# dash-robotics/perception

Measured on AMD Instinct MI355X. Metric: frames/sec (640x480 D435 cloud, plane+cluster+ICP), higher is better.
Workload: dtype f32

## Files before the change

### perception_amd/csrc/k_icp_lat.hip

```cpp
#include "kernels.hpp"
#include "icp_solve_row.hpp"
#include "lat_search.hpp"

namespace cd {

#ifdef CD_LAT_TIMERS
__device__ unsigned long long g_lat_stats[8];
extern "C" int cd_debug_lat_stats(unsigned long long* out, int reset) {
    if (hipMemcpyFromSymbol(out, HIP_SYMBOL(g_lat_stats), sizeof(g_lat_stats)) != hipSuccess) return -1;
    if (reset) { unsigned long long z[8] = {0}; (void)hipMemcpyToSymbol(HIP_SYMBOL(g_lat_stats), z, sizeof(z)); }
    return 0;
}
#define LAT_T(k) { const long long tn_ = clock64(); tph[k] += tn_ - tlast; tlast = tn_; }
#else
#define LAT_T(k)
#endif

struct LatSlot {
    int k, src_off, n, tslot;
    int phase;
    int gen;
    int ready;
    int pad;
};
enum { LAT_ITER = 0, LAT_FIT = 1, LAT_EMPTY = 2 };

#ifndef CD_LAT_SOLVE_ROW
#define CD_LAT_SOLVE_ROW 1
#endif
#ifndef CD_LAT_WAVES_PER_EU
#define CD_LAT_WAVES_PER_EU 4
#endif
template <int CPW, int WPC, bool BOUNDED>
__global__ void __launch_bounds__(CPW * WPC * WAVE, CD_LAT_WAVES_PER_EU)
k_icp_lat(int nitems, const int* __restrict__ order, const IcpCluster* __restrict__ cl, IcpState* __restrict__ st,
          unsigned long long* __restrict__ accf, const IcpLattice* __restrict__ lats, float4* __restrict__ src,
          const float4* __restrict__ src0, int* __restrict__ queue, unsigned long long* __restrict__ busy,
          unsigned long long* __restrict__ busy_out, IcpParams prm, IcpBound bnd) {
    __shared__ float4 s_tab[CPW][LAT_MAX_TAB];
    __shared__ int4 s_face[CPW][2 * LAT_MAX_FACES];
    __shared__ unsigned long long s_acc[CPW][16];
    __shared__ IcpState s_so[CPW];
    __shared__ LatSlot s_slot[CPW];
    __shared__ int s_flags[2];
    __shared__ unsigned s_nv[BOUNDED ? CPW : 1];
    const int lane = threadIdx.x & 63, wave = threadIdx.x >> 6;
    const int slot = wave / WPC, sub = wave % WPC;
    const long long wg_t0 = wall_clock64();
    auto refill = [&](int s) {
        LatSlot& sl = s_slot[s];
        for (int i = 0; i < 16; ++i) s_acc[s][i] = 0ull;
        if constexpr (BOUNDED) s_nv[s] = 0u;
        sl.ready = 0;
        for (;;) {
            const int item = atomicAdd(queue, 1);
            if (item >= nitems) { sl.phase = LAT_EMPTY; return; }
            const int k = order[item];
            if (st[2 * (size_t)k].done) continue;
            const IcpCluster c = cl[k];
            sl.k = k; sl.src_off = c.src_off; sl.n = c.n; sl.tslot = c.slot;
            s_so[s] = st[2 * (size_t)k];
            sl.phase = LAT_ITER;
            sl.gen += 1;
            return;
        }
    };
    if (threadIdx.x < CPW) { s_slot[threadIdx.x].gen = 0; refill(threadIdx.x); }
    if (threadIdx.x == 0) { s_flags[0] = 0; s_flags[1] = 1; }
    __syncthreads();
    int my_gen = 0;
#ifdef CD_LAT_TIMERS
    long long tph[6] = {0, 0, 0, 0, 0, 0}, tlast = clock64();
#endif
    for (;;) {
        if (s_flags[1]) {
            const LatSlot sl = s_slot[slot];
            const bool mine = sl.phase != LAT_EMPTY && sl.gen != my_gen;
            if (mine) {
                const IcpLattice* __restrict__ L = lats + sl.tslot;
                for (int i = sub * WAVE + lane; i < L->ntab; i += WPC * WAVE) s_tab[slot][i] = L->tab[i];
                if (sub == 0 && lane < LAT_MAX_FACES) {
                    const int f = lane, w = L->w[f], u = L->fast[f], v = 3 - w - u;
                    s_face[slot][f] = make_int4(w, u, L->base[f], __float_as_int(L->c[f]));
                    s_face[slot][LAT_MAX_FACES + f] = make_int4(L->toff[u], L->toff[v < 0 || v > 2 ? 0 : v], L->n[u], 0);
                }
                my_gen = sl.gen;
            }
            __syncthreads();
        }
        LAT_T(5)
        {
            const int phase = __builtin_amdgcn_readfirstlane(s_slot[slot].phase), n = __builtin_amdgcn_readfirstlane(s_slot[slot].n);
            const int src_off = __builtin_amdgcn_readfirstlane(s_slot[slot].src_off), tslot = __builtin_amdgcn_readfirstlane(s_slot[slot].tslot);
            const int npass = (n + 63) >> 6;
            float4* pts = src + src_off;
            const float4* tab = s_tab[slot];
            const int4* face = s_face[slot];
            LatFaces F;
            {
                const IcpLattice* __restrict__ L = lats + (phase == LAT_EMPTY ? 0 : tslot);
                lat_faces_load(L, F);
            }
            const bool nf3 = F.nface <= 3;
            if (phase == LAT_ITER) {
                const bool moved = s_so[slot].iters > 0;
                float T[12];
#pragma unroll
                for (int i = 0; i < 12; ++i) T[i] = s_so[slot].T[i];
                unsigned long long S[16];
#pragma unroll
                for (int i = 0; i < 16; ++i) S[i] = 0ull;
                unsigned nv = 0u;
                float4 pnext = pts[min((sub << 6) + lane, n - 1)];
                for (int pss = sub; pss < npass; pss += WPC) {
                    const int myq = (pss << 6) + lane;
                    const bool act = myq < n;
                    const float4 p = pnext;
                    pnext = pts[min(((pss + WPC) << 6) + lane, n - 1)];
                    float px = p.x, py = p.y, pz = p.z;
                    if (moved) {
                        xform(T, p.x, p.y, p.z, px, py, pz);
                        if (act) pts[myq] = make_float4(px, py, pz, p.w);
                    }
                    const LatHit h = F.axes ? lat_nearest_axes<true>(tab, face, F, px, py, pz)
                                            : (nf3 ? lat_nearest<true, 3>(tab, face, F, px, py, pz) : lat_nearest<true, LAT_MAX_FACES>(tab, face, F, px, py, pz));
                    const bool keep = act && (!BOUNDED || h.d <= bnd.d2_max);
                    if constexpr (BOUNDED) nv += (unsigned)__popcll(ballot64(keep));
                    if (keep) {
                        const float pv[3] = {px, py, pz}, qv[3] = {h.nx, h.ny, h.nz};
                        const float big_c = fmaxf(fmaxf(fmaxf(fabsf(px), fabsf(py)), fabsf(pz)), fmaxf(fmaxf(fabsf(h.nx), fabsf(h.ny)), fabsf(h.nz)));
                        if (big_c < 256.f && h.d < 16384.f) {
#pragma unroll
                            for (int a = 0; a < 3; ++a) {
                                S[a] += LatFix<FIX_SHIFT>::bits(pv[a]);
                                S[3 + a] += LatFix<FIX_SHIFT>::bits(qv[a]);
#pragma unroll
                                for (int b = 0; b < 3; ++b) S[6 + 3 * a + b] += LatFix<FIX_SHIFT>::bits(__fmul_rn(qv[a], pv[b]));
                            }
                            S[15] += LatFix<FIX_SHIFT_D2>::bits(h.d);
                        } else {
#pragma unroll
                            for (int a = 0; a < 3; ++a) {
                                S[a] += (unsigned long long)fixq(pv[a], FIX_SHIFT) + LatFix<FIX_SHIFT>::C;
                                S[3 + a] += (unsigned long long)fixq(qv[a], FIX_SHIFT) + LatFix<FIX_SHIFT>::C;
#pragma unroll
                                for (int b = 0; b < 3; ++b) S[6 + 3 * a + b] += (unsigned long long)fixq(__fmul_rn(qv[a], pv[b]), FIX_SHIFT) + LatFix<FIX_SHIFT>::C;
                            }
                            S[15] += (unsigned long long)fixq(h.d, FIX_SHIFT_D2) + LatFix<FIX_SHIFT_D2>::C;
                        }
                    }
                }
                if (sub < npass) wave_fold_to_lds(S, 16, s_acc[slot]);
                if constexpr (BOUNDED) { if (sub < npass && lane == 0) atomicAdd(&s_nv[slot], nv); }
                if (sub == 0 && lane == 0) s_slot[slot].ready = 1;
            } else if (phase == LAT_FIT) {
                const float4* pts0 = src0 + src_off;
                float T[12], Tf[12];
#pragma unroll
                for (int i = 0; i < 12; ++i) {
                    T[i] = __int_as_float(__builtin_amdgcn_readfirstlane(__float_as_int(s_so[slot].T[i])));
                    Tf[i] = __int_as_float(__builtin_amdgcn_readfirstlane(__float_as_int(s_so[slot].Tfinal[i])));
                }
                unsigned long long S[16];
#pragma unroll
                for (int i = 0; i < 16; ++i) S[i] = 0ull;
                float4 pnext = pts[min((sub << 6) + lane, n - 1)], p0next = pts0[min((sub << 6) + lane, n - 1)];
                for (int pss = sub; pss < npass; pss += WPC) {
                    const int myq = (pss << 6) + lane;
                    const bool act = myq < n;
                    const float4 p = pnext, p0 = p0next;
                    pnext = pts[min(((pss + WPC) << 6) + lane, n - 1)];
                    p0next = pts0[min(((pss + WPC) << 6) + lane, n - 1)];
                    float ox, oy, oz;
                    xform(T, p.x, p.y, p.z, ox, oy, oz);
                    if (act) pts[myq] = make_float4(ox, oy, oz, p.w);
                    float qx, qy, qz;
                    xform(Tf, p0.x, p0.y, p0.z, qx, qy, qz);
                    const LatHit h = F.axes ? lat_nearest_axes<false>(tab, face, F, qx, qy, qz)
                                            : (nf3 ? lat_nearest<false, 3>(tab, face, F, qx, qy, qz) : lat_nearest<false, LAT_MAX_FACES>(tab, face, F, qx, qy, qz));
                    if (act) S[0] += h.d < 16384.f ? LatFix<FIX_SHIFT_D2>::bits(h.d) : (unsigned long long)fixq(h.d, FIX_SHIFT_D2) + LatFix<FIX_SHIFT_D2>::C;
                }
                if (sub < npass) wave_fold_to_lds(S, 1, s_acc[slot]);
            }
        }
        LAT_T(0)
        if (threadIdx.x == 0) s_flags[1] = 0;
        __syncthreads();
        LAT_T(1)
#if CD_LAT_SOLVE_ROW
        const int tid = (int)threadIdx.x | s_flags[0];
        if (tid < CPW * 16) {
            const int s = tid >> 4, l = tid & 15;
            LatSlot& sl = s_slot[s];
            const int phase = sl.phase, ready = sl.ready;
            const int nv = BOUNDED && phase == LAT_ITER ? (int)s_nv[s] : sl.n;
            const unsigned long long off = (unsigned long long)nv * LatFix<FIX_SHIFT>::C, off_d = (unsigned long long)nv * LatFix<FIX_SHIFT_D2>::C;
            if (phase == LAT_ITER && ready) {
                RowLanes row(tid);
                RowLanes::V<unsigned long long> a;
                a.v = s_acc[s][l] - (l == 15 ? off_d : off);
                const int done = icp_step_row<BOUNDED>(row, s_so[s], a, nv, prm);
                s_acc[s][l] = 0ull;
                if (l == 0) {
                    if (done) sl.phase = LAT_FIT;
                    if constexpr (BOUNDED) s_nv[s] = 0u;
                    sl.ready = 0;
                }
            } else if (phase == LAT_FIT && l == 0) {
                s_so[s].done = 1;
                st[2 * (size_t)sl.k] = s_so[s];
                st[2 * (size_t)sl.k + 1] = s_so[s];
                accf[sl.k] = s_acc[s][0] - off_d;
                refill(s);
                if (sl.phase != LAT_EMPTY) s_flags[1] = 1;
            }
        }
#else
        if (threadIdx.x < CPW) {
            const int s = threadIdx.x;
            LatSlot& sl = s_slot[s];
            const int nv = BOUNDED && sl.phase == LAT_ITER ? (int)s_nv[s] : sl.n;
            const unsigned long long off = (unsigned long long)nv * LatFix<FIX_SHIFT>::C, off_d = (unsigned long long)nv * LatFix<FIX_SHIFT_D2>::C;
            if (sl.phase == LAT_ITER && sl.ready) {
                for (int i = 0; i < 15; ++i) s_acc[s][i] -= off;
                s_acc[s][15] -= off_d;
                if (icp_step<BOUNDED>(s_so[s], s_acc[s], nv, prm)) sl.phase = LAT_FIT;
                for (int i = 0; i < 16; ++i) s_acc[s][i] = 0ull;
                if constexpr (BOUNDED) s_nv[s] = 0u;
                sl.ready = 0;
            } else if (sl.phase == LAT_FIT) {
                s_so[s].done = 1;
                st[2 * (size_t)sl.k] = s_so[s];
                st[2 * (size_t)sl.k + 1] = s_so[s];
                accf[sl.k] = s_acc[s][0] - off_d;
                refill(s);
                if (sl.phase != LAT_EMPTY) s_flags[1] = 1;
            }
        }
#endif
        LAT_T(2)
        __syncthreads();
        LAT_T(3)
#ifdef CD_LAT_TIMERS
        tph[4] += 1;
#endif
        int all_empty = 1;
#pragma unroll
        for (int s = 0; s < CPW; ++s) all_empty &= s_slot[s].phase == LAT_EMPTY ? 1 : 0;
        if (all_empty) break;
    }
#ifdef CD_LAT_TIMERS
    if (threadIdx.x == 0) for (int i = 0; i < 6; ++i) atomicAdd(&g_lat_stats[i], (unsigned long long)tph[i]);
#endif
    if (threadIdx.x == 0 && busy) {
        atomicAdd(busy, (unsigned long long)(wall_clock64() - wg_t0) * (unsigned long long)(CPW * WPC));
        if (busy_out) {
            __threadfence();
            if (atomicAdd(queue + 1, 1) == (int)gridDim.x - 1) {
                __threadfence();
                *busy_out = atomicAdd(busy, 0ull);
            }
        }
    }
}

__device__ __forceinline__ bool lat_same_bits(float a, float b) { return __float_as_uint(a) == __float_as_uint(b); }

__global__ void __launch_bounds__(BLOCK) k_lat_nn(const IcpLattice* __restrict__ L, const float4* __restrict__ q, int n, int* __restrict__ out_idx,
                                                  float* __restrict__ out_d2) {
    __shared__ float4 s_tab[LAT_MAX_TAB];
    __shared__ int4 s_face[2 * LAT_MAX_FACES];
    LatFaces F;
    lat_stage<BLOCK>(L, F, s_tab, s_face);
    for (int base = blockIdx.x * BLOCK; base < n; base += gridDim.x * BLOCK) {
        const int i = base + threadIdx.x;
        const float4 p = q[i < n ? i : n - 1];
        const LatHit h = lat_nearest<true, LAT_MAX_FACES, true>(s_tab, s_face, F, p.x, p.y, p.z);
        const LatHit g = lat_nearest<false, 3>(s_tab, s_face, F, p.x, p.y, p.z);
        bool same = F.nface > 3 || h.d == g.d;
        const int idx = lat_index(s_face, F, h);
        if (F.axes) {
            const LatHit a = lat_nearest_axes<true, true>(s_tab, s_face, F, p.x, p.y, p.z);
            const LatHit b = lat_nearest_axes<false>(s_tab, s_face, F, p.x, p.y, p.z);
            same = same && a.d == h.d && b.d == h.d && lat_same_bits(a.nx, h.nx) && lat_same_bits(a.ny, h.ny) && lat_same_bits(a.nz, h.nz) &&
                   lat_index(s_face, F, a) == idx;
        }
        if (i < n) { out_idx[i] = idx; out_d2[i] = same ? h.d : __uint_as_float(0x7fc00000u); }
    }
}

template <int CPW, int WPC>
static void launch_lat_shape(hipStream_t s, int nitems, int n_wg, const int* order, const IcpCluster* cl, IcpState* st, unsigned long long* accf,
                             const IcpLattice* lats, float4* src, const float4* src0, int* queue, unsigned long long* busy, unsigned long long* busy_out,
                             IcpParams prm, const IcpBound& bnd) {
    if (bnd.bounded)
        hipLaunchKernelGGL((k_icp_lat<CPW, WPC, true>), dim3(n_wg), dim3(CPW * WPC * WAVE), 0, s, nitems, order, cl, st, accf, lats, src, src0, queue, busy, busy_out, prm, bnd);
    else
        hipLaunchKernelGGL((k_icp_lat<CPW, WPC, false>), dim3(n_wg), dim3(CPW * WPC * WAVE), 0, s, nitems, order, cl, st, accf, lats, src, src0, queue, busy, busy_out, prm, bnd);
}
void launch_icp_lat(hipStream_t s, int nitems, int cpw, int wpc, int n_wg, const IcpProblems& P, const IcpTemplates& T, const IcpScratch& S,
                    unsigned long long* busy, unsigned long long* busy_out, IcpParams prm, const IcpBound& bnd) {
    if (nitems <= 0 || n_wg <= 0) return;
#define CD_LAT_CASE(C, W) if (cpw == C && wpc == W) return launch_lat_shape<C, W>(s, nitems, n_wg, P.order, P.cl, P.st, P.accf, T.lats, S.src, S.src0, S.queue, busy, busy_out, prm, bnd);
    CD_LAT_CASE(1, 1) CD_LAT_CASE(1, 2) CD_LAT_CASE(1, 4) CD_LAT_CASE(1, 8) CD_LAT_CASE(1, 16)
    CD_LAT_CASE(2, 1) CD_LAT_CASE(2, 2) CD_LAT_CASE(2, 4)
    CD_LAT_CASE(4, 1) CD_LAT_CASE(4, 2) CD_LAT_CASE(4, 4)
    CD_LAT_CASE(8, 1) CD_LAT_CASE(8, 2)
#undef CD_LAT_CASE
    launch_lat_shape<1, 4>(s, nitems, n_wg, P.order, P.cl, P.st, P.accf, T.lats, S.src, S.src0, S.queue, busy, busy_out, prm, bnd);
}
void launch_lat_nn(hipStream_t s, const IcpLattice* lat, const float4* q, int n, int* out_idx, float* out_d2) {
    if (n <= 0) return;
    const int g = (n + BLOCK - 1) / BLOCK;
    hipLaunchKernelGGL(k_lat_nn, dim3(g < 1024 ? g : 1024), dim3(BLOCK), 0, s, lat, q, n, out_idx, out_d2);
}

}
```

Baseline: 209,900.

## Balance lattice ICP passes across all waves in the workgroup instead of per slot

Replaces the fixed mapping, where each slot owned WPC waves and those waves split only that cluster's 64-point passes, with a global partition. The total pass count across all CPW slots is split evenly across every wave in the workgroup, so a wave can cover parts of several clusters. The goal is to stop waves idling when cluster sizes differ or a slot is empty. In exchange it adds a per-iteration loop over slots, per-segment face loads and LDS folds, and drops the ready flag so the solve runs every iteration for each ITER slot.

Result: no change. 210,400, median of 5 (+0.2%).

```diff
diff --git a/perception_amd/csrc/k_icp_lat.hip b/perception_amd/csrc/k_icp_lat.hip
--- a/perception_amd/csrc/k_icp_lat.hip
+++ b/perception_amd/csrc/k_icp_lat.hip
@@ -1,6 +1,7 @@
 #include "kernels.hpp"
 #include "icp_solve_row.hpp"
 #include "lat_search.hpp"
+#include "lat_balance.hpp"
 
 namespace cd {
 
@@ -12,18 +13,20 @@
     return 0;
 }
 #define LAT_T(k) { const long long tn_ = clock64(); tph[k] += tn_ - tlast; tlast = tn_; }
+#define LAT_WAIT(stmt) { const long long tb_ = clock64(); stmt; twait += clock64() - tb_; }
 #else
 #define LAT_T(k)
+#define LAT_WAIT(stmt) stmt;
 #endif
 
 struct LatSlot {
     int k, src_off, n, tslot;
     int phase;
     int gen;
-    int ready;
-    int pad;
+    int pad[2];
 };
 enum { LAT_ITER = 0, LAT_FIT = 1, LAT_EMPTY = 2 };
+static_assert(lat_passes(LAT_ITER, 65) == 2 && lat_passes(LAT_FIT, 64) == 1 && lat_passes(LAT_EMPTY, 64) == 0, "lat_balance.hpp's phase words");
 
 #ifndef CD_LAT_SOLVE_ROW
 #define CD_LAT_SOLVE_ROW 1
@@ -46,12 +49,12 @@
     __shared__ unsigned s_nv[BOUNDED ? CPW : 1];
     const int lane = threadIdx.x & 63, wave = threadIdx.x >> 6;
     const int slot = wave / WPC, sub = wave % WPC;
+    const int wave_u = __builtin_amdgcn_readfirstlane(wave);
     const long long wg_t0 = wall_clock64();
     auto refill = [&](int s) {
         LatSlot& sl = s_slot[s];
         for (int i = 0; i < 16; ++i) s_acc[s][i] = 0ull;
         if constexpr (BOUNDED) s_nv[s] = 0u;
-        sl.ready = 0;
         for (;;) {
             const int item = atomicAdd(queue, 1);
             if (item >= nitems) { sl.phase = LAT_EMPTY; return; }
@@ -70,7 +73,7 @@
     __syncthreads();
     int my_gen = 0;
 #ifdef CD_LAT_TIMERS
-    long long tph[6] = {0, 0, 0, 0, 0, 0}, tlast = clock64();
+    long long tph[6] = {0, 0, 0, 0, 0, 0}, tlast = clock64(), twait = 0;
 #endif
     for (;;) {
         if (s_flags[1]) {
@@ -90,112 +93,123 @@
         }
         LAT_T(5)
         {
-            const int phase = __builtin_amdgcn_readfirstlane(s_slot[slot].phase), n = __builtin_amdgcn_readfirstlane(s_slot[slot].n);
-            const int src_off = __builtin_amdgcn_readfirstlane(s_slot[slot].src_off), tslot = __builtin_amdgcn_readfirstlane(s_slot[slot].tslot);
-            const int npass = (n + 63) >> 6;
-            float4* pts = src + src_off;
-            const float4* tab = s_tab[slot];
-            const int4* face = s_face[slot];
-            LatFaces F;
-            {
-                const IcpLattice* __restrict__ L = lats + (phase == LAT_EMPTY ? 0 : tslot);
-                lat_faces_load(L, F);
-            }
-            const bool nf3 = F.nface <= 3;
-            if (phase == LAT_ITER) {
-                const bool moved = s_so[slot].iters > 0;
-                float T[12];
-#pragma unroll
-                for (int i = 0; i < 12; ++i) T[i] = s_so[slot].T[i];
-                unsigned long long S[16];
-#pragma unroll
-                for (int i = 0; i < 16; ++i) S[i] = 0ull;
-                unsigned nv = 0u;
-                float4 pnext = pts[min((sub << 6) + lane, n - 1)];
-                for (int pss = sub; pss < npass; pss += WPC) {
-                    const int myq = (pss << 6) + lane;
-                    const bool act = myq < n;
-                    const float4 p = pnext;
-                    pnext = pts[min(((pss + WPC) << 6) + lane, n - 1)];
-                    float px = p.x, py = p.y, pz = p.z;
-                    if (moved) {
-                        xform(T, p.x, p.y, p.z, px, py, pz);
-                        if (act) pts[myq] = make_float4(px, py, pz, p.w);
-                    }
-                    const LatHit h = F.axes ? lat_nearest_axes<true>(tab, face, F, px, py, pz)
-                                            : (nf3 ? lat_nearest<true, 3>(tab, face, F, px, py, pz) : lat_nearest<true, LAT_MAX_FACES>(tab, face, F, px, py, pz));
-                    const bool keep = act && (!BOUNDED || h.d <= bnd.d2_max);
-                    if constexpr (BOUNDED) nv += (unsigned)__popcll(ballot64(keep));
-                    if (keep) {
-                        const float pv[3] = {px, py, pz}, qv[3] = {h.nx, h.ny, h.nz};
-                        const float big_c = fmaxf(fmaxf(fmaxf(fabsf(px), fabsf(py)), fabsf(pz)), fmaxf(fmaxf(fabsf(h.nx), fabsf(h.ny)), fabsf(h.nz)));
-                        if (big_c < 256.f && h.d < 16384.f) {
-#pragma unroll
-                            for (int a = 0; a < 3; ++a) {
-                                S[a] += LatFix<FIX_SHIFT>::bits(pv[a]);
-                                S[3 + a] += LatFix<FIX_SHIFT>::bits(qv[a]);
-#pragma unroll
-                                for (int b = 0; b < 3; ++b) S[6 + 3 * a + b] += LatFix<FIX_SHIFT>::bits(__fmul_rn(qv[a], pv[b]));
+            int P = 0;
+#pragma unroll
+            for (int s = 0; s < CPW; ++s) P += lat_passes(__builtin_amdgcn_readfirstlane(s_slot[s].phase), __builtin_amdgcn_readfirstlane(s_slot[s].n));
+            LatBalance bal(P, CPW * WPC, wave_u);
+#pragma unroll 1
+            for (int s = 0; s < CPW && (CPW == 1 || bal.base < bal.hi); ++s) {
+                const int phase = __builtin_amdgcn_readfirstlane(s_slot[s].phase), n = __builtin_amdgcn_readfirstlane(s_slot[s].n);
+                constexpr int STEP = CPW == 1 ? WPC : 1;
+                int first, end;
+                if constexpr (CPW == 1) {
+                    first = wave_u; end = lat_passes(phase, n);
+                    if (first >= end) continue;
+                } else {
+                    if (!bal.next(lat_passes(phase, n), first, end)) continue;
+                }
+                const int src_off = __builtin_amdgcn_readfirstlane(s_slot[s].src_off), tslot = __builtin_amdgcn_readfirstlane(s_slot[s].tslot);
+                float4* pts = src + src_off;
+                const float4* tab = s_tab[s];
+                const int4* face = s_face[s];
+                LatFaces F;
+                lat_faces_load(lats + tslot, F);
+                const bool nf3 = F.nface <= 3;
+                if (phase == LAT_ITER) {
+                    const bool moved = s_so[s].iters > 0;
+                    float T[12];
+#pragma unroll
+                    for (int i = 0; i < 12; ++i) T[i] = s_so[s].T[i];
+                    unsigned long long S[16];
+#pragma unroll
+                    for (int i = 0; i < 16; ++i) S[i] = 0ull;
+                    unsigned nv = 0u;
+                    float4 pnext = pts[min((first << 6) + lane, n - 1)];
+                    for (int pss = first; pss < end; pss += STEP) {
+                        const int myq = (pss << 6) + lane;
+                        const bool act = myq < n;
+                        const float4 p = pnext;
+                        pnext = pts[min(((CPW == 1 ? pss + STEP : min(pss + 1, end - 1)) << 6) + lane, n - 1)];
+                        float px = p.x, py = p.y, pz = p.z;
+                        if (moved) {
+                            xform(T, p.x, p.y, p.z, px, py, pz);
+                            if (act) pts[myq] = make_float4(px, py, pz, p.w);
+                        }
+                        const LatHit h = F.axes ? lat_nearest_axes<true>(tab, face, F, px, py, pz)
+                                                : (nf3 ? lat_nearest<true, 3>(tab, face, F, px, py, pz) : lat_nearest<true, LAT_MAX_FACES>(tab, face, F, px, py, pz));
+                        const bool keep = act && (!BOUNDED || h.d <= bnd.d2_max);
+                        if constexpr (BOUNDED) nv += (unsigned)__popcll(ballot64(keep));
+                        if (keep) {
+                            const float pv[3] = {px, py, pz}, qv[3] = {h.nx, h.ny, h.nz};
+                            const float big_c = fmaxf(fmaxf(fmaxf(fabsf(px), fabsf(py)), fabsf(pz)), fmaxf(fmaxf(fabsf(h.nx), fabsf(h.ny)), fabsf(h.nz)));
+                            if (big_c < 256.f && h.d < 16384.f) {
+#pragma unroll
+                                for (int a = 0; a < 3; ++a) {
+                                    S[a] += LatFix<FIX_SHIFT>::bits(pv[a]);
+                                    S[3 + a] += LatFix<FIX_SHIFT>::bits(qv[a]);
+#pragma unroll
+                                    for (int b = 0; b < 3; ++b) S[6 + 3 * a + b] += LatFix<FIX_SHIFT>::bits(__fmul_rn(qv[a], pv[b]));
+                                }
+                                S[15] += LatFix<FIX_SHIFT_D2>::bits(h.d);
+                            } else {
+#pragma unroll
+                                for (int a = 0; a < 3; ++a) {
+                                    S[a] += (unsigned long long)fixq(pv[a], FIX_SHIFT) + LatFix<FIX_SHIFT>::C;
+                                    S[3 + a] += (unsigned long long)fixq(qv[a], FIX_SHIFT) + LatFix<FIX_SHIFT>::C;
+#pragma unroll
+                                    for (int b = 0; b < 3; ++b) S[6 + 3 * a + b] += (unsigned long long)fixq(__fmul_rn(qv[a], pv[b]), FIX_SHIFT) + LatFix<FIX_SHIFT>::C;
+                                }
+                                S[15] += (unsigned long long)fixq(h.d, FIX_SHIFT_D2) + LatFix<FIX_SHIFT_D2>::C;
                             }
-                            S[15] += LatFix<FIX_SHIFT_D2>::bits(h.d);
-                        } else {
-#pragma unroll
-                            for (int a = 0; a < 3; ++a) {
-                                S[a] += (unsigned long long)fixq(pv[a], FIX_SHIFT) + LatFix<FIX_SHIFT>::C;
-                                S[3 + a] += (unsigned long long)fixq(qv[a], FIX_SHIFT) + LatFix<FIX_SHIFT>::C;
-#pragma unroll
-                                for (int b = 0; b < 3; ++b) S[6 + 3 * a + b] += (unsigned long long)fixq(__fmul_rn(qv[a], pv[b]), FIX_SHIFT) + LatFix<FIX_SHIFT>::C;
-                            }
-                            S[15] += (unsigned long long)fixq(h.d, FIX_SHIFT_D2) + LatFix<FIX_SHIFT_D2>::C;
                         }
                     }
+                    wave_fold_to_lds(S, 16, s_acc[s]);
+                    if constexpr (BOUNDED) { if (lane == 0) atomicAdd(&s_nv[s], nv); }
+                } else {
+                    const float4* pts0 = src0 + src_off;
+                    float T[12], Tf[12];
+#pragma unroll
+                    for (int i = 0; i < 12; ++i) {
+                        T[i] = __int_as_float(__builtin_amdgcn_readfirstlane(__float_as_int(s_so[s].T[i])));
+                        Tf[i] = __int_as_float(__builtin_amdgcn_readfirstlane(__float_as_int(s_so[s].Tfinal[i])));
+                    }
+                    unsigned long long S[16];
+#pragma unroll
+                    for (int i = 0; i < 16; ++i) S[i] = 0ull;
+                    float4 pnext = pts[min((first << 6) + lane, n - 1)], p0next = pts0[min((first << 6) + lane, n - 1)];
+                    for (int pss = first; pss < end; pss += STEP) {
+                        const int myq = (pss << 6) + lane;
+                        const bool act = myq < n;
+                        const float4 p = pnext, p0 = p0next;
+                        const int nq = min(((CPW == 1 ? pss + STEP : min(pss + 1, end - 1)) << 6) + lane, n - 1);
+                        pnext = pts[nq];
+                        p0next = pts0[nq];
+                        float ox, oy, oz;
+                        xform(T, p.x, p.y, p.z, ox, oy, oz);
+                        if (act) pts[myq] = make_float4(ox, oy, oz, p.w);
+                        float qx, qy, qz;
+                        xform(Tf, p0.x, p0.y, p0.z, qx, qy, qz);
+                        const LatHit h = F.axes ? lat_nearest_axes<false>(tab, face, F, qx, qy, qz)
+                                                : (nf3 ? lat_nearest<false, 3>(tab, face, F, qx, qy, qz) : lat_nearest<false, LAT_MAX_FACES>(tab, face, F, qx, qy, qz));
+                        if (act) S[0] += h.d < 16384.f ? LatFix<FIX_SHIFT_D2>::bits(h.d) : (unsigned long long)fixq(h.d, FIX_SHIFT_D2) + LatFix<FIX_SHIFT_D2>::C;
+                    }
+                    wave_fold_to_lds(S, 1, s_acc[s]);
                 }
-                if (sub < npass) wave_fold_to_lds(S, 16, s_acc[slot]);
-                if constexpr (BOUNDED) { if (sub < npass && lane == 0) atomicAdd(&s_nv[slot], nv); }
-                if (sub == 0 && lane == 0) s_slot[slot].ready = 1;
-            } else if (phase == LAT_FIT) {
-                const float4* pts0 = src0 + src_off;
-                float T[12], Tf[12];
-#pragma unroll
-                for (int i = 0; i < 12; ++i) {
-                    T[i] = __int_as_float(__builtin_amdgcn_readfirstlane(__float_as_int(s_so[slot].T[i])));
-                    Tf[i] = __int_as_float(__builtin_amdgcn_readfirstlane(__float_as_int(s_so[slot].Tfinal[i])));
-                }
-                unsigned long long S[16];
-#pragma unroll
-                for (int i = 0; i < 16; ++i) S[i] = 0ull;
-                float4 pnext = pts[min((sub << 6) + lane, n - 1)], p0next = pts0[min((sub << 6) + lane, n - 1)];
-                for (int pss = sub; pss < npass; pss += WPC) {
-                    const int myq = (pss << 6) + lane;
-                    const bool act = myq < n;
-                    const float4 p = pnext, p0 = p0next;
-                    pnext = pts[min(((pss + WPC) << 6) + lane, n - 1)];
-                    p0next = pts0[min(((pss + WPC) << 6) + lane, n - 1)];
-                    float ox, oy, oz;
-                    xform(T, p.x, p.y, p.z, ox, oy, oz);
-                    if (act) pts[myq] = make_float4(ox, oy, oz, p.w);
-                    float qx, qy, qz;
-                    xform(Tf, p0.x, p0.y, p0.z, qx, qy, qz);
-                    const LatHit h = F.axes ? lat_nearest_axes<false>(tab, face, F, qx, qy, qz)
-                                            : (nf3 ? lat_nearest<false, 3>(tab, face, F, qx, qy, qz) : lat_nearest<false, LAT_MAX_FACES>(tab, face, F, qx, qy, qz));
-                    if (act) S[0] += h.d < 16384.f ? LatFix<FIX_SHIFT_D2>::bits(h.d) : (unsigned long long)fixq(h.d, FIX_SHIFT_D2) + LatFix<FIX_SHIFT_D2>::C;
-                }
-                if (sub < npass) wave_fold_to_lds(S, 1, s_acc[slot]);
             }
         }
         LAT_T(0)
         if (threadIdx.x == 0) s_flags[1] = 0;
-        __syncthreads();
+        LAT_WAIT(__syncthreads())
         LAT_T(1)
 #if CD_LAT_SOLVE_ROW
         const int tid = (int)threadIdx.x | s_flags[0];
         if (tid < CPW * 16) {
             const int s = tid >> 4, l = tid & 15;
             LatSlot& sl = s_slot[s];
-            const int phase = sl.phase, ready = sl.ready;
+            const int phase = sl.phase;
             const int nv = BOUNDED && phase == LAT_ITER ? (int)s_nv[s] : sl.n;
             const unsigned long long off = (unsigned long long)nv * LatFix<FIX_SHIFT>::C, off_d = (unsigned long long)nv * LatFix<FIX_SHIFT_D2>::C;
-            if (phase == LAT_ITER && ready) {
+            if (phase == LAT_ITER) {
                 RowLanes row(tid);
                 RowLanes::V<unsigned long long> a;
                 a.v = s_acc[s][l] - (l == 15 ? off_d : off);
@@ -204,7 +218,6 @@
                 if (l == 0) {
                     if (done) sl.phase = LAT_FIT;
                     if constexpr (BOUNDED) s_nv[s] = 0u;
-                    sl.ready = 0;
                 }
             } else if (phase == LAT_FIT && l == 0) {
                 s_so[s].done = 1;
@@ -221,13 +234,12 @@
             LatSlot& sl = s_slot[s];
             const int nv = BOUNDED && sl.phase == LAT_ITER ? (int)s_nv[s] : sl.n;
             const unsigned long long off = (unsigned long long)nv * LatFix<FIX_SHIFT>::C, off_d = (unsigned long long)nv * LatFix<FIX_SHIFT_D2>::C;
-            if (sl.phase == LAT_ITER && sl.ready) {
+            if (sl.phase == LAT_ITER) {
                 for (int i = 0; i < 15; ++i) s_acc[s][i] -= off;
                 s_acc[s][15] -= off_d;
                 if (icp_step<BOUNDED>(s_so[s], s_acc[s], nv, prm)) sl.phase = LAT_FIT;
                 for (int i = 0; i < 16; ++i) s_acc[s][i] = 0ull;
                 if constexpr (BOUNDED) s_nv[s] = 0u;
-                sl.ready = 0;
             } else if (sl.phase == LAT_FIT) {
                 s_so[s].done = 1;
                 st[2 * (size_t)sl.k] = s_so[s];
@@ -251,6 +263,7 @@
     }
 #ifdef CD_LAT_TIMERS
     if (threadIdx.x == 0) for (int i = 0; i < 6; ++i) atomicAdd(&g_lat_stats[i], (unsigned long long)tph[i]);
+    if (lane == 0) { atomicAdd(&g_lat_stats[6], (unsigned long long)twait); atomicAdd(&g_lat_stats[7], (unsigned long long)tph[4]); }
 #endif
     if (threadIdx.x == 0 && busy) {
         atomicAdd(busy, (unsigned long long)(wall_clock64() - wg_t0) * (unsigned long long)(CPW * WPC));
diff --git a/perception_amd/csrc/lat_balance.hpp b/perception_amd/csrc/lat_balance.hpp
--- /dev/null
+++ b/perception_amd/csrc/lat_balance.hpp
@@ -0,0 +1,33 @@
+#pragma once
+
+#if defined(__HIPCC__) || defined(__CUDACC__)
+#define CD_LAT_HD __host__ __device__ __forceinline__
+#else
+#define CD_LAT_HD inline
+#endif
+
+namespace cd {
+
+CD_LAT_HD constexpr int lat_passes(int phase, int n) { return (phase == 0 || phase == 1) && n > 0 ? (int)(((unsigned)n + 63u) >> 6) : 0; }
+
+CD_LAT_HD constexpr int lat_balance_cut(int P, int W, int w) {
+    const int q = P / W, r = P - q * W;
+    return w * q + (w * r) / W;
+}
+
+struct LatBalance {
+    int lo, hi;
+    int base;
+    int slot;
+    CD_LAT_HD LatBalance(int P, int W, int w) : lo(lat_balance_cut(P, W, w)), hi(lat_balance_cut(P, W, w + 1)), base(0), slot(-1) {}
+    CD_LAT_HD bool next(int np, int& first, int& end) {
+        const int a = lo - base, b = hi - base;
+        first = a > 0 ? a : 0;
+        end = b < np ? b : np;
+        base += np;
+        slot += 1;
+        return first < end;
+    }
+};
+
+}
diff --git a/perception_amd/csrc/lat_balance_check.cpp b/perception_amd/csrc/lat_balance_check.cpp
--- /dev/null
+++ b/perception_amd/csrc/lat_balance_check.cpp
@@ -0,0 +1,114 @@
+#include <cstdint>
+#include <cstdio>
+#include <cstring>
+#include <vector>
+
+#include "lat_balance.hpp"
+
+using cd::LatBalance;
+
+struct Seg { int slot, first, end; };
+
+static uint64_t rng_state = 0x9e3779b97f4a7c15ull;
+static uint32_t rnd() {
+    uint64_t z = (rng_state += 0x9e3779b97f4a7c15ull);
+    z = (z ^ (z >> 30)) * 0xbf58476d1ce4e5b9ull;
+    z = (z ^ (z >> 27)) * 0x94d049bb133111ebull;
+    return (uint32_t)((z ^ (z >> 31)) >> 32);
+}
+
+struct Totals { long cases = 0, failures = 0; int max_segments = 0, max_straddling = 0; };
+
+static void fail(Totals& t, const char* what, int W, const std::vector<int>& np, int w) {
+    if (t.failures < 20) {
+        std::fprintf(stderr, "FAIL %s: W %d wave %d np", what, W, w);
+        for (int v : np) std::fprintf(stderr, " %d", v);
+        std::fprintf(stderr, "\n");
+    }
+    t.failures += 1;
+}
+
+static void one_case(const std::vector<int>& np, int W, bool dump, Totals& t) {
+    const int C = (int)np.size();
+    int P = 0;
+    for (int v : np) P += v;
+    t.cases += 1;
+    if (dump) {
+        std::printf("%d |", W);
+        for (int v : np) std::printf(" %d", v);
+        std::printf(" |");
+    }
+    std::vector<std::pair<int, int>> want, got;
+    for (int s = 0; s < C; ++s) for (int p = 0; p < np[s]; ++p) want.push_back({s, p});
+    int prev_hi = 0, min_size = INT32_MAX, max_size = 0, straddling = 0;
+    for (int w = 0; w < W; ++w) {
+        LatBalance bal(P, W, w);
+        const int lo = bal.lo, hi = bal.hi;
+        if (lo != prev_hi || hi < lo) fail(t, "ranges are not disjoint and contiguous", W, np, w);
+        prev_hi = hi;
+        if (hi - lo < min_size) min_size = hi - lo;
+        if (hi - lo > max_size) max_size = hi - lo;
+        std::vector<Seg> segs;
+        for (int s = 0; s < C; ++s) {
+            int first = -1, end = -1;
+            const bool some = bal.next(np[s], first, end);
+            if (bal.slot != s) fail(t, "slot counter", W, np, w);
+            if (some) {
+                if (first < 0 || end > np[s] || first >= end) fail(t, "segment outside its slot", W, np, w);
+                segs.push_back(Seg{s, first, end});
+            }
+        }
+        if (bal.base != P) fail(t, "base after the last slot", W, np, w);
+        int covered = 0;
+        for (const Seg& g : segs) {
+            covered += g.end - g.first;
+            for (int p = g.first; p < g.end; ++p) got.push_back({g.slot, p});
+        }
+        if (covered != hi - lo) fail(t, "segments do not add up to the range", W, np, w);
+        if (hi == lo && !segs.empty()) fail(t, "segment of an empty range", W, np, w);
+        if ((int)segs.size() > C) fail(t, "more segments than slots", W, np, w);
+        if ((int)segs.size() > t.max_segments) t.max_segments = (int)segs.size();
+        if (segs.size() > 1) straddling += 1;
+        if (dump) {
+            std::printf(" %d %d :", lo, hi);
+            for (size_t i = 0; i < segs.size(); ++i) std::printf("%s %d %d %d", i ? "," : "", segs[i].slot, segs[i].first, segs[i].end);
+            std::printf("%s", w + 1 < W ? " ;" : "\n");
+        }
+    }
+    if (prev_hi != P) fail(t, "ranges do not cover [0, P)", W, np, -1);
+    if (max_size - min_size > 1) fail(t, "range sizes differ by more than one", W, np, -1);
+    if (got != want) fail(t, "segments do not enumerate every (slot, pass) once, in order", W, np, -1);
+    if (P == 0 && !got.empty()) fail(t, "segments with nothing to do", W, np, -1);
+    if (straddling > (C > 1 ? C - 1 : 0)) fail(t, "more straddling waves than slot boundaries", W, np, -1);
+    if (straddling > t.max_straddling) t.max_straddling = straddling;
+}
+
+int main(int argc, char** argv) {
+    const bool dump = argc > 1 && !std::strcmp(argv[1], "--dump");
+    static const int VALUES[7] = {0, 1, 2, 3, 11, 22, 68};
+    static const int WAVES[5] = {1, 2, 4, 8, 16};
+    Totals t;
+    for (int C : {1, 2, 4}) {
+        int total = 1;
+        for (int i = 0; i < C; ++i) total *= 7;
+        for (int code = 0; code < total; ++code) {
+            std::vector<int> np(C);
+            for (int i = 0, c = code; i < C; ++i, c /= 7) np[i] = VALUES[c % 7];
+            for (int W : WAVES) one_case(np, W, dump, t);
+        }
+    }
+    for (int k = 0; k < 4000; ++k) {
+        std::vector<int> np(8);
+        const bool sparse = k & 1;
+        for (int i = 0; i < 8; ++i) np[i] = sparse ? (rnd() % 4 == 0 ? (int)(rnd() % 4) : 0) : (rnd() % 5 == 0 ? 0 : (int)(rnd() % 300));
+        for (int W : WAVES) one_case(np, W, dump, t);
+    }
+    for (int W : WAVES) for (int w = 0; w <= W; ++w) for (int P : {0, 1, 15, 16, 17, 1 << 20, (1 << 28) - 1, 1 << 28}) {
+        t.cases += 1;
+        if (cd::lat_balance_cut(P, W, w) != (int)(((long long)w * P) / W)) { t.failures += 1; std::fprintf(stderr, "FAIL cut P %d W %d w %d\n", P, W, w); }
+    }
+    static_assert(cd::lat_passes(0, 1) == 1 && cd::lat_passes(0, 64) == 1 && cd::lat_passes(1, 65) == 2 && cd::lat_passes(2, 640) == 0 && cd::lat_passes(0, 0) == 0 &&
+                  cd::lat_passes(1, 2147483647) == 33554432, "lat_passes");
+    if (!dump) std::printf("{\"cases\": %ld, \"failures\": %ld, \"max_segments\": %d, \"max_straddling_waves\": %d}\n", t.cases, t.failures, t.max_segments, t.max_straddling);
+    return t.failures ? 1 : 0;
+}
```
